# 123-code/Distributed-neural-networks

Measured on AMD Instinct MI355X. Metric: images/sec CIFAR-10 2-stage, higher is better.
Workload: dtype fp32 (bf16x3 split emulation, ~2^-16 per product); 1 GPU; model=cifar10-convnet (cifar_model_parts.py NeuralNetwork), global_batch=65536, parallelism=pp2-colocated, stages=2, microbatches=1, stage0_spare_cus=0, p2p=none, stage_cut=conv|fc (reference split, 16 KiB/img hop)

## Files before the change

csrc/bindings.cpp:

```cpp
#include <pybind11/pybind11.h>
#include <pybind11/stl.h>
#include <hip/hip_runtime.h>
#include <cstdint>

#include "kernels/api.h"
#include "comm/p2p.h"

#include <string>
#include <vector>

namespace py = pybind11;
#define P(x) reinterpret_cast<void*>(static_cast<uintptr_t>(x))
#define CP(x) reinterpret_cast<const void*>(static_cast<uintptr_t>(x))
#define FP(x) reinterpret_cast<float*>(static_cast<uintptr_t>(x))
#define CFP(x) reinterpret_cast<const float*>(static_cast<uintptr_t>(x))
#define IP(x) reinterpret_cast<int*>(static_cast<uintptr_t>(x))
#define CIP(x) reinterpret_cast<const int*>(static_cast<uintptr_t>(x))
#define ST(x) reinterpret_cast<hipStream_t>(static_cast<uintptr_t>(x))
typedef uint64_t u64;

PYBIND11_MODULE(_dnn_hip, m) {
  m.doc() = "distributed_neural_networks_amd HIP/CDNA4 kernels (gfx950)";
  m.attr("arch") = "gfx950";

// ... 62 lines not shown
                          int act, u64 qo, int ldq, u64 sxo, int kpo, u64 st) {
    return dnn_gemm_fp8_mx(CP(a), CP(sx), CP(w), CFP(sw), P(c), ldc, CFP(bias), CP(r), ldr, M, N, Kb, act, P(qo), ldq,
                           P(sxo), kpo, ST(st));
  });
  m.def("gemm_fp8_qkv_scatter_mx", [](u64 a, u64 sx, u64 w, u64 sw, u64 bias, u64 q, u64 kc, u64 vc, u64 pos, int B,
                                      int T, int H, int Hkv, int hd, int S, int Kb, u64 st) {
    return dnn_gemm_fp8_qkv_scatter_mx(CP(a), CP(sx), CP(w), CFP(sw), CFP(bias), P(q), P(kc), P(vc),
                                       reinterpret_cast<const int*>(static_cast<uintptr_t>(pos)), B, T, H, Hkv, hd, S,
                                       Kb, ST(st));
  });
  m.def("argmax_final", [](u64 part, int S, int M, u64 out, u64 out2, u64 pos_inc, u64 st, u64 hist, int hist_ld) {
    return dnn_argmax_final(CP(part), S, M, IP(out), IP(out2), IP(pos_inc), ST(st), IP(hist), hist_ld);
  });
  m.def("gemm_oneshot_sweep", [](u64 A, int lda, u64 Wsh, u64 sw, u64 C, int ldc, int M, int N, int K, int mt, int ntw,
                                 int steps, int splitk, int w8, u64 ws, long long ws_bytes, u64 st) {
    return dnn_gemm_oneshot_sweep(CP(A), lda, CP(Wsh), CFP(sw), P(C), ldc, M, N, K, mt, ntw, steps, splitk, w8, P(ws),
                                  ws_bytes, ST(st));
  });
  m.def("gemm_skinny_sweep", [](u64 A, int lda, u64 W, int ldw, u64 sw, u64 C, int ldc, int M, int N, int K, int nt,
                                int u, int ks, int pipe, int w8, u64 st) {
    return dnn_gemm_skinny_sweep(CP(A), lda, CP(W), ldw, CFP(sw), P(C), ldc, M, N, K, nt, u, ks, pipe, w8, ST(st));
  });
  m.def("gemm_set_tile", [](int tile) { return dnn_gemm_set_tile(tile); });
  m.def("gemm_set_anatomy", [](int bits) { return dnn_gemm_set_anatomy(bits); });
  m.def("gemm_set_skinny_pin", [](int id, int ks, int n, int k) { return dnn_gemm_set_skinny_pin(id, ks, n, k); });
  m.def("gemm_set_half_cost", [](float c) { return dnn_gemm_set_half_cost(c); });
  m.def("gemm_bf16_qkv_scatter", [](u64 A, int lda, u64 W, int ldw, u64 bias, u64 rowstat, u64 colsum, u64 q, u64 kc,
                                    u64 vc, u64 pos, int B, int T, int H, int Hkv, int hd, int S, int K, u64 st) {
    return dnn_gemm_bf16_qkv_scatter(CP(A), lda, CP(W), ldw, CFP(bias), CFP(rowstat), CFP(colsum), P(q), P(kc), P(vc),
                                     CIP(pos), B, T, H, Hkv, hd, S, K, ST(st));
  });
  m.def("gemm_fp8_qkv_scatter", [](u64 A8, u64 sa, u64 W8, u64 sw, u64 bias, u64 q, u64 kc, u64 vc, u64 pos, int B,
                                   int T, int H, int Hkv, int hd, int S, int Kb, u64 st) {
    return dnn_gemm_fp8_qkv_scatter(CP(A8), CFP(sa), CP(W8), CFP(sw), CFP(bias), P(q), P(kc), P(vc), CIP(pos), B, T, H,
                                    Hkv, hd, S, Kb, ST(st));
  });
  m.def("gemm_set_res_prefetch", [](int on) { return dnn_gemm_set_res_prefetch(on); });
  m.def("gemm_set_skinny_max_m", [](int m) { return dnn_gemm_set_skinny_max_m(m); });
  m.def("gemm_fp8_set_tile", [](int tile) { return dnn_gemm_fp8_set_tile(tile); });
  m.def("silu_mul_packed", [](u64 gu, int ld_in, u64 out, int ld_out, int M, int F, u64 st) {
    return dnn_silu_mul_packed(CP(gu), ld_in, P(out), ld_out, M, F, ST(st));
  });
  m.def("cifar_stage0_v4", [](u64 x, u64 out, u64 w1p, u64 b1, u64 w2p, u64 b2, int B, int grid, u64 st) {
    return dnn_cifar_stage0_v4(CFP(x), P(out), CP(w1p), CFP(b1), CP(w2p), CFP(b2), B, grid, ST(st));
  });
  m.def("cifar_set_v4_pt", [](int pt) { return dnn_cifar_set_v4_pt(pt); });
  m.def("cifar_stage0_x3", [](u64 x, u64 out, u64 w1h, u64 w1l, u64 b1, u64 w2h, u64 w2l, u64 b2, int B, int grid,
                              u64 st, int split_out) {
    return dnn_cifar_stage0_x3(CFP(x), FP(out), CP(w1h), CP(w1l), CFP(b1), CP(w2h), CP(w2l), CFP(b2), B, grid,
                               ST(st), split_out);
  }, py::arg("x"), py::arg("out"), py::arg("w1h"), py::arg("w1l"), py::arg("b1"), py::arg("w2h"), py::arg("w2l"),
        py::arg("b2"), py::arg("B"), py::arg("grid"), py::arg("st"), py::arg("split_out") = 0);
  m.def("cifar_s0_set_wide_store", [](int on) { return dnn_cifar_s0_set_wide_store(on); });
  m.def("cifar_split3", [](u64 a, int lda, u64 o, int ldo, int M, int K, u64 st, int blocked) {
    return dnn_cifar_split3(CFP(a), lda, P(o), ldo, M, K, ST(st), blocked);
  }, py::arg("a"), py::arg("lda"), py::arg("o"), py::arg("ldo"), py::arg("M"), py::arg("K"), py::arg("st"),
        py::arg("blocked") = 0);
  m.def("cifar_fc1_x3", [](u64 a, int lda, u64 wh, u64 wl, int ldw, u64 bias, u64 c, int ldc, int M, int N, int K,
                           u64 st, int a_split) {
    return dnn_cifar_fc1_x3(CFP(a), lda, CP(wh), CP(wl), ldw, CFP(bias), FP(c), ldc, M, N, K, ST(st), a_split);
  }, py::arg("a"), py::arg("lda"), py::arg("wh"), py::arg("wl"), py::arg("ldw"), py::arg("bias"), py::arg("c"),
        py::arg("ldc"), py::arg("M"), py::arg("N"), py::arg("K"), py::arg("st"), py::arg("a_split") = 0);
  m.def("cifar_split_blocked", [](u64 a, u64 o, int M, int K, int dir, u64 st) {
    return dnn_cifar_split_blocked(CFP(a), FP(o), M, K, dir, ST(st));
  });
  m.def("cifar_head_tail_x3", [](u64 hid, u64 w2h, u64 w2l, u64 b2, u64 probs, u64 pred, int B, u64 st) {
    return dnn_cifar_head_tail_x3(CFP(hid), CP(w2h), CP(w2l), CFP(b2), FP(probs), IP(pred), B, ST(st));
  });
  m.def("cifar_head_tail", [](u64 hid, u64 w2p, u64 b2, u64 probs, u64 pred, int B, u64 st) {
    return dnn_cifar_head_tail(CP(hid), CP(w2p), CFP(b2), FP(probs), IP(pred), B, ST(st));
  });
#ifdef DNN_HAVE_TRANSFORMER
  m.def("row_stats", [](u64 x, int ldx, u64 stats, int M, int N, float eps, int rms, u64 st) {
    return dnn_row_stats(CP(x), ldx, FP(stats), M, N, eps, rms, ST(st));
  });
  m.def("layernorm", [](u64 x, int ldx, u64 w, u64 b, u64 y, int ldy, int M, int N, float eps, int rms, u64 st) {
    return dnn_layernorm(CP(x), ldx, CFP(w), CFP(b), P(y), ldy, M, N, eps, rms, ST(st));
  });
  m.def("layernorm_q8", [](u64 x, int ldx, u64 w, u64 b, u64 q, int ldq, u64 sq, int M, int N, int kpad, float eps,
                           int rms, u64 st, int split) {
    return dnn_layernorm_q8(CP(x), ldx, CFP(w), CFP(b), P(q), ldq, FP(sq), M, N, kpad, eps, rms, ST(st), split);
  }, py::arg("x"), py::arg("ldx"), py::arg("w"), py::arg("b"), py::arg("q"), py::arg("ldq"), py::arg("sq"), py::arg("M"),
     py::arg("N"), py::arg("kpad"), py::arg("eps"), py::arg("rms"), py::arg("st"), py::arg("split") = 0);
  m.def("embed_gpt2", [](u64 idx, u64 wte, u64 wpe, u64 out, int B, int T, int d, u64 pos, int V, int Pn, u64 st) {
    return dnn_embed_gpt2(CIP(idx), CP(wte), CP(wpe), P(out), B, T, d, CIP(pos), V, Pn, ST(st));
  });
  m.def("qkv_split", [](u64 qkv, u64 q, u64 kc, u64 vc, int B, int T, int H, int Hkv, int hd, int S, u64 pos,
                        u64 cos, u64 sin, int rope, u64 st, int kv8) {
    return dnn_qkv_split(CP(qkv), P(q), P(kc), P(vc), B, T, H, Hkv, hd, S, CIP(pos), CFP(cos), CFP(sin), rope,
                         ST(st), kv8);
  }, py::arg("qkv"), py::arg("q"), py::arg("kc"), py::arg("vc"), py::arg("B"), py::arg("T"), py::arg("H"),
     py::arg("Hkv"), py::arg("hd"), py::arg("S"), py::arg("pos"), py::arg("cos"), py::arg("sin"), py::arg("rope"),
     py::arg("st"), py::arg("kv8") = 0);
  m.def("flash_attn_qkv", [](u64 qkv, int ldqkv, u64 kc, u64 vc, u64 o, int B, int T, int H, int Hkv, int hd, int S,
                             u64 pos, float scale, u64 st, int kv8) {
    return dnn_flash_attn_qkv(CP(qkv), ldqkv, P(kc), P(vc), P(o), B, T, H, Hkv, hd, S, CIP(pos), scale, ST(st), kv8);
  }, py::arg("qkv"), py::arg("ldqkv"), py::arg("kc"), py::arg("vc"), py::arg("o"), py::arg("B"), py::arg("T"),
     py::arg("H"), py::arg("Hkv"), py::arg("hd"), py::arg("S"), py::arg("pos"), py::arg("scale"), py::arg("st"),
     py::arg("kv8") = 0);
  m.def("flash_attn", [](u64 q, u64 kc, u64 vc, u64 o, int B, int T, int H, int Hkv, int hd, int S, u64 pos,
                         float scale, u64 st, int kv8) {
    return dnn_flash_attn(CP(q), CP(kc), CP(vc), P(o), B, T, H, Hkv, hd, S, CIP(pos), scale, ST(st), kv8);
  }, py::arg("q"), py::arg("kc"), py::arg("vc"), py::arg("o"), py::arg("B"), py::arg("T"), py::arg("H"),
     py::arg("Hkv"), py::arg("hd"), py::arg("S"), py::arg("pos"), py::arg("scale"), py::arg("st"), py::arg("kv8") = 0);
  m.def("attn_decode", [](u64 q, u64 kc, u64 vc, u64 o, int B, int H, int Hkv, int hd, int S, u64 lens,
                          float scale, int splits, u64 ws, u64 st, int kv8) {
// ... 79 lines not shown
```

csrc/kernels/api.h:

```cpp
#pragma once
#include <hip/hip_runtime.h>

extern "C" {
int dnn_gemm_bf16(const void* A, int lda, const void* W, int ldw, void* C, int ldc, const float* bias, const void* R,
                  int ldr, int M, int N, int K, int act, int out_f32, hipStream_t st, const void* Wsh = nullptr,
                  const float* rowstat = nullptr, const float* colsum = nullptr, void* ws = nullptr,
                  long long ws_bytes = 0);
int dnn_row_stats(const void* x, int ldx, float* stats, int M, int N, float eps, int rms, hipStream_t st);
int dnn_gemm_set_tile(int tile);
int dnn_gemm_set_anatomy(int bits);
int dnn_gemm_set_skinny_pin(int id, int ks, int n, int k);
int dnn_gemm_bf16_qkv_scatter(const void* A, int lda, const void* W, int ldw, const float* bias, const float* rowstat,
                              const float* colsum, void* q, void* kc, void* vc, const int* pos, int B, int T, int H,
                              int Hkv, int hd, int S, int K, hipStream_t st);
int dnn_gemm_fp8_qkv_scatter(const void* A8, const float* sa, const void* W8, const float* sw, const float* bias,
                             void* q, void* kc, void* vc, const int* pos, int B, int T, int H, int Hkv, int hd, int S,
                             int Kb, hipStream_t st);
int dnn_gemm_set_res_prefetch(int on);
int dnn_gemm_set_half_cost(float c);
int dnn_gemm_set_skinny_max_m(int m);
int dnn_gemm_fp8_set_tile(int tile);
int dnn_gemm_fp8_256(const void* A, const float* sa, const void* W, const float* sw, void* C, int ldc, const float* bias,
                     const void* R, int ldr, int M, int N, int Kb, int act, hipStream_t st);
int dnn_gemm_skinny_sweep(const void* A, int lda, const void* W, int ldw, const float* sw, void* C, int ldc, int M,
                          int N, int K, int nt, int u, int ks, int pipe, int w8, hipStream_t st);
int dnn_gemm_skinny_norm(const void* A, int lda, const void* W, int ldw, void* C, int ldc, const float* bias,
                         const void* R, int ldr, int M, int N, int K, int act, int norm, const float* colsum, float eps,
                         hipStream_t st, const void* Wsh = nullptr, void* ws = nullptr, long long ws_bytes = 0);
int dnn_gemm_skinny_w8(const void* A, int lda, const void* W, int ldw, const float* sw, void* C, int ldc,
                       const float* bias, const void* R, int ldr, int M, int N, int K, int act, int norm,
                       const float* colsum, float eps, hipStream_t st, const void* Wsh = nullptr, void* ws = nullptr,
                       long long ws_bytes = 0);
int dnn_gemm_skinny(const void* A, int lda, const float* sa, const void* W, int ldw, const float* sw, void* C, int ldc,
                    const float* bias, const void* R, int ldr, int M, int N, int K, int act, int out_f32, int fp8,
                    hipStream_t st, const void* Wsh = nullptr, void* ws = nullptr, long long ws_bytes = 0);
int dnn_gemm_set_stream(int on, long long min_bytes, int fold = -1);
int dnn_gemm_set_oneshot(int on, int mt, int ntw, int steps, int splitk);
int dnn_gemm_set_oneshot_lds_floor(int bytes);
int dnn_gemm_set_oneshot_probe(void* rec, int abl);
int dnn_gemm_oneshot_sweep(const void* A, int lda, const void* Wsh, const float* sw, void* C, int ldc, int M, int N,
                           int K, int mt, int ntw, int steps, int splitk, int w8, void* ws, long long ws_bytes,
                           hipStream_t st);
int dnn_gemm_set_head(int on);
int dnn_gemm_head(const void* A, int lda, const void* Wsh, const float* sw, const float* colsum, const float* bias,
                  float eps, int norm, void* C, int ldc, int M, int N, int K, int w8, void* part, int part_cap,
                  hipStream_t st);
int dnn_argmax_final(const void* part, int S, int M, int* out, int* out2, int* pos_inc, hipStream_t st,
                     int* hist = nullptr, int hist_ld = 0);
int dnn_gemm_set_split_tail(int on);
int dnn_quant_fp8_mx(const void* x, int ldx, void* q, int ldq, void* sx, int M, int K, int kpad, hipStream_t st);
int dnn_layernorm_q8_mx(const void* x, int ldx, const float* w, const float* b, void* q, int ldq, void* sx, int M,
                        int N, int kpad, float eps, int rms, hipStream_t st);
int dnn_gemm_fp8_mx(const void* A8, const void* sx, const void* W8, const float* sw, void* C, int ldc,
                    const float* bias, const void* R, int ldr, int M, int N, int Kb, int act, void* qo, int ldq,
                    void* sxo, int kpo, hipStream_t st);
int dnn_gemm_fp8_qkv_scatter_mx(const void* A8, const void* sx, const void* W8, const float* sw, const float* bias,
                                void* q, void* kc, void* vc, const int* pos, int B, int T, int H, int Hkv, int hd,
                                int S, int Kb, hipStream_t st);
int dnn_gemm_rowstats(void* out, int out_ld, const void* in, int in_ld);
int dnn_gemm_rowstats_written();
int dnn_gemm_set_epi_prefetch(int on);
int dnn_gemm_oneshot_ablate(const void* A, int lda, const void* Wsh, const float* sw, void* C, int ldc, int M, int N,
                            int K, int cfg, int abl, hipStream_t st);
int dnn_silu_mul_packed(const void* gu, int ld_in, void* out, int ld_out, int M, int F, hipStream_t st);
int dnn_cifar_stage0_v4(const float* x, void* out, const void* w1p, const float* b1, const void* w2p, const float* b2,
                        int B, int grid, hipStream_t st);
int dnn_cifar_set_v4_pt(int pt);
int dnn_cifar_stage0_x3(const float* x, float* out, const void* w1h, const void* w1l, const float* b1, const void* w2h,
                        const void* w2l, const float* b2, int B, int grid, hipStream_t st, int split_out = 0);
int dnn_cifar_s0_set_wide_store(int on);
int dnn_cifar_split3(const float* a, int lda, void* o, int ldo, int M, int K, hipStream_t st, int blocked = 0);
int dnn_cifar_fc1_x3(const float* A, int lda, const void* Wh, const void* Wl, int ldw, const float* bias, float* C,
                     int ldc, int M, int N, int K, hipStream_t st, int a_split = 0);
int dnn_cifar_split_blocked(const float* a, float* o, int M, int K, int dir, hipStream_t st);
int dnn_cifar_head_tail_x3(const float* hid, const void* w2h, const void* w2l, const float* b2, float* probs, int* pred,
                           int B, hipStream_t st);
int dnn_cifar_head_tail(const void* hid, const void* w2p, const float* b2, float* probs, int* pred, int B,
                        hipStream_t st);
int dnn_layernorm_q8(const void* x, int ldx, const float* w, const float* b, void* q, int ldq, float* sq, int M, int N,
                     int kpad, float eps, int rms, hipStream_t st, int split = 0);
int dnn_layernorm(const void* x, int ldx, const float* w, const float* b, void* y, int ldy, int M, int N, float eps,
                  int rms, hipStream_t st);
int dnn_embed_gpt2(const int* idx, const void* wte, const void* wpe, void* out, int B, int T, int d, const int* pos,
                   int V, int P, hipStream_t st);
int dnn_qkv_split(const void* qkv, void* q, void* kc, void* vc, int B, int T, int H, int Hkv, int hd, int S,
                  const int* pos, const float* cos, const float* sin, int rope, hipStream_t st, int kv8 = 0);
int dnn_flash_attn_qkv(const void* qkv, int ldqkv, void* kc, void* vc, void* o, int B, int T, int H, int Hkv,
                       int hd, int S, const int* pos, float scale, hipStream_t st, int kv8 = 0);
int dnn_flash_attn(const void* q, const void* kc, const void* vc, void* o, int B, int T, int H, int Hkv, int hd, int S,
                   const int* pos, float scale, hipStream_t st, int kv8 = 0);
int dnn_attn_decode_qkv(const void* qkv, int ldqkv, void* kc, void* vc, void* o, int B, int H, int Hkv, int hd, int S,
                        const int* pos, const float* cosT, const float* sinT, float scale, int splits, float* ws,
                        hipStream_t st, int kv8 = 0);
int dnn_attn_decode(const void* q, const void* kc, const void* vc, void* o, int B, int H, int Hkv, int hd, int S,
                    const int* lens, float scale, int splits, float* ws, hipStream_t st, int kv8 = 0);
int dnn_sample_topk(const void* x, int ld, int M, int N, int* out, float temperature, int topk, unsigned seed,
                    const int* step, hipStream_t st);
int dnn_argmax_rows(const void* x, int ld, int M, int N, int* out, int f32in, hipStream_t st, int* out2 = nullptr,
                    int* pos_inc = nullptr, void* part = nullptr, int* hist = nullptr, int hist_ld = 0);
int dnn_quant_fp8_rows(const void* x, int ldx, void* q, float* scale, int M, int K, int kpad, hipStream_t st,
                       int split = 0);
int dnn_gemm_fp8(const void* A, const float* sa, const void* W, const float* sw, void* C, int ldc, const float* bias,
                 const void* R, int ldr, int M, int N, int K, int act, hipStream_t st);
}
```

csrc/kernels/cifar_x3.hip:

```cpp
#include <type_traits>

#include "gemm_epilogue.h"

namespace dnn {
namespace x3 {

__device__ __forceinline__ void split2(float a, float b, uint32_t& hi, uint32_t& lo) {
  hi = pack2bf(a, b);
  const float ah = __uint_as_float(hi << 16), bh = __uint_as_float(hi & 0xffff0000u);
  lo = pack2bf(a - ah, b - bh);
}

__device__ __forceinline__ int dpp_xor1(int v) { return __builtin_amdgcn_mov_dpp(v, 0xB1, 0xF, 0xF, false); }
__device__ __forceinline__ int dpp_xor2(int v) { return __builtin_amdgcn_mov_dpp(v, 0x4E, 0xF, 0xF, false); }

constexpr int XW = 40;
constexpr int XPL = 34 * XW * 8;
constexpr int A1PL = 18 * 18 * 64;
constexpr int A1_OFF = 4 * XPL;
constexpr int LDS_BYTES = A1_OFF + 4 * A1PL;

__device__ __forceinline__ int xin_off(int k, int lo) { return ((k & 1) * 2 + lo) * XPL; }
__device__ __forceinline__ int a1_off(int k, int lo) { return A1_OFF + ((k & 1) * 2 + lo) * A1PL; }

template <int S, int I, int LO>
__device__ __forceinline__ constexpr int c2_imm() {
  return (8 * I + (S >> 1) % 3) * 64 + LO * A1PL;
}

template <int S>
__device__ __forceinline__ void c2_issue(const uint32_t (&b)[3][2], bf16x8 (&a)[4]) {
  constexpr int ky = (S >> 1) / 3, par = S & 1;
  asm volatile("ds_read_b128 %0, %1 offset:%2" : "=v"(a[0]) : "v"(b[ky][par]), "i"(c2_imm<S, 0, 0>()));
  asm volatile("ds_read_b128 %0, %1 offset:%2" : "=v"(a[1]) : "v"(b[ky][par]), "i"(c2_imm<S, 1, 0>()));
  asm volatile("ds_read_b128 %0, %1 offset:%2" : "=v"(a[2]) : "v"(b[ky][par]), "i"(c2_imm<S, 0, 1>()));
  asm volatile("ds_read_b128 %0, %1 offset:%2" : "=v"(a[3]) : "v"(b[ky][par]), "i"(c2_imm<S, 1, 1>()));
}

template <int S>
__device__ __forceinline__ void c2_step(const uint32_t (&b)[3][2], const bf16x8 (&wh)[18], const bf16x8 (&wl)[18],
                                        f32x16 (&acc)[2], bf16x8 (&cur)[4], bf16x8 (&nxt)[4]) {
  if constexpr (S + 1 < 18) {
    c2_issue<S + 1>(b, nxt);
    asm volatile("s_waitcnt lgkmcnt(4)" ::: "memory");
  } else {
    asm volatile("s_waitcnt lgkmcnt(0)" ::: "memory");
  }
  __builtin_amdgcn_sched_barrier(0);
  acc[0] = __builtin_amdgcn_mfma_f32_32x32x16_bf16(cur[0], wh[S], acc[0], 0, 0, 0);
  acc[1] = __builtin_amdgcn_mfma_f32_32x32x16_bf16(cur[1], wh[S], acc[1], 0, 0, 0);
  acc[0] = __builtin_amdgcn_mfma_f32_32x32x16_bf16(cur[0], wl[S], acc[0], 0, 0, 0);
  acc[1] = __builtin_amdgcn_mfma_f32_32x32x16_bf16(cur[1], wl[S], acc[1], 0, 0, 0);
  acc[0] = __builtin_amdgcn_mfma_f32_32x32x16_bf16(cur[2], wh[S], acc[0], 0, 0, 0);
  acc[1] = __builtin_amdgcn_mfma_f32_32x32x16_bf16(cur[3], wh[S], acc[1], 0, 0, 0);
  __builtin_amdgcn_sched_barrier(0);
  if constexpr (S + 1 < 18) c2_step<S + 1>(b, wh, wl, acc, nxt, cur);
}

template <int N>
__device__ __forceinline__ void resident_fence(const bf16x8 (&w)[N]) {
#pragma unroll
  for (int i = 0; i < N; ++i) asm volatile("" ::"v"(w[i]));
}

}

using namespace x3;

template <bool WIDE, bool SPLIT_OUT>
__global__ __launch_bounds__(512, 1) void cifar_stage0_x3_kernel(
    const float* __restrict__ x, float* __restrict__ out, const bf16_t* __restrict__ w1h,
    const bf16_t* __restrict__ w1l, const float* __restrict__ b1, const bf16_t* __restrict__ w2h,
    const bf16_t* __restrict__ w2l, const float* __restrict__ b2, int B) {
  __shared__ __attribute__((aligned(16))) char smem[LDS_BYTES];
  const int tid = threadIdx.x, lane = tid & 63;
  const int wave = __builtin_amdgcn_readfirstlane(tid >> 6);
  const bool producer = wave < 4;
  const int rw = wave & 3;
  const int rt = tid & 255;
  const int h = lane >> 5, r32 = lane & 31;
  const int n = B > (int)blockIdx.x ? (B - 1 - (int)blockIdx.x) / (int)gridDim.x + 1 : 0;

  for (int i = tid; i < LDS_BYTES / 16; i += 512) reinterpret_cast<uint4*>(smem)[i] = make_uint4(0, 0, 0, 0);

  __syncthreads();

  if (producer) {
    bf16x8 w1hf[3], w1lf[3];
#pragma unroll
    for (int s = 0; s < 3; ++s) {
      w1hf[s] = *reinterpret_cast<const bf16x8*>(w1h + r32 * 48 + s * 16 + h * 8);
      w1lf[s] = *reinterpret_cast<const bf16x8*>(w1l + r32 * 48 + s * 16 + h * 8);
    }
    const float bias = b1[r32];
    resident_fence(w1hf);
    resident_fence(w1lf);
    asm volatile("" ::"v"(bias));

    float pf[4][3];
    auto load_img = [&](int k) {
      const float* xb = x + (size_t)(blockIdx.x + (size_t)k * gridDim.x) * 3072;
#pragma unroll
      for (int i = 0; i < 4; ++i)
#pragma unroll
        for (int c = 0; c < 3; ++c) pf[i][c] = xb[c * 1024 + rt + 256 * i];
    };
    auto stage_img = [&](int k) {
      char* xh = smem + xin_off(k, 0);
      char* xl = smem + xin_off(k, 1);
#pragma unroll
      for (int i = 0; i < 4; ++i) {
        const int p = rt + 256 * i, yy = p >> 5, xx = p & 31;
        uint2 vh, vl;
        split2(pf[i][0], pf[i][1], vh.x, vl.x);
        split2(pf[i][2], 0.f, vh.y, vl.y);
        const int o = ((yy + 1) * XW + xx + 1) * 8;
        *reinterpret_cast<uint2*>(xh + o) = vh;
        *reinterpret_cast<uint2*>(xl + o) = vl;
      }
    };
    const int c1_lane = ((r32 >> 3) * XW + (r32 & 7) + 2 * h) * 8;
    const int q = ((r32 & 1) ? 2 : 0) + ((r32 & 2) ? 1 : 0);
    const int cb = r32 & ~3;

    auto conv1_epi = [&](int t, const f32x16& acc, int k) {
      const int ty = t >> 2, tx = t & 3;
      float v[4];
#pragma unroll
      for (int qy = 0; qy < 2; ++qy)
#pragma unroll
        for (int qx = 0; qx < 2; ++qx) {
          const int g0 = (2 * qy) * 4 + 2 * qx;
          v[qy * 2 + qx] = fmaxf(fmax_nan(fmax_nan(acc[g0], acc[g0 + 1]), fmax_nan(acc[g0 + 4], acc[g0 + 5])) + bias, 0.f);
        }
      const bool odd = r32 & 1;
      const int s0 = __float_as_int(odd ? v[0] : v[2]), s1 = __float_as_int(odd ? v[1] : v[3]);
      const float r0 = __int_as_float(dpp_xor1(s0)), r1 = __int_as_float(dpp_xor1(s1));
      uint32_t u0h, u0l, u1h, u1l;
      if (!odd) {
        split2(v[0], r0, u0h, u0l);
        split2(v[1], r1, u1h, u1l);
      } else {
        split2(r0, v[2], u0h, u0l);
        split2(r1, v[3], u1h, u1l);
      }
      const bool hi2 = r32 & 2;
      const uint32_t rch = (uint32_t)dpp_xor2((int)(hi2 ? u0h : u1h));
      const uint32_t rcl = (uint32_t)dpp_xor2((int)(hi2 ? u0l : u1l));
      const uint32_t mh = hi2 ? u1h : u0h, ml = hi2 ? u1l : u0l;
      uint2 wh, wl;
      wh.x = hi2 ? rch : mh;
      wh.y = hi2 ? mh : rch;
      wl.x = hi2 ? rcl : ml;
      wl.y = hi2 ? ml : rcl;
      const int Y = 2 * ty + (q >> 1) + 1, X = 4 * tx + 2 * h + (q & 1) + 1;
      const int o = (Y * 18 + X) * 64 + ((((cb >> 3) ^ (Y & 3))) << 4) + (cb & 7) * 2;
      *reinterpret_cast<uint2*>(smem + a1_off(k, 0) + o) = wh;
      *reinterpret_cast<uint2*>(smem + a1_off(k, 1) + o) = wl;
    };
    auto frag = [&](const char* p) {
      const uint2 a = *reinterpret_cast<const uint2*>(p);
      const uint2 b = *reinterpret_cast<const uint2*>(p + 8);
      return __builtin_bit_cast(bf16x8, make_uint4(a.x, a.y, b.x, b.y));
    };
    auto conv1_pair = [&](int ta, int tb, int k) {
      const char* xh = smem + xin_off(k, 0);
      const int oa = c1_lane + ((4 * (ta >> 2)) * XW + 8 * (ta & 3)) * 8;
      const int ob = c1_lane + ((4 * (tb >> 2)) * XW + 8 * (tb & 3)) * 8;
      bf16x8 fah[3], fal[3], fbh[3], fbl[3];
#pragma unroll
      for (int s = 0; s < 3; ++s) {
        fah[s] = frag(xh + oa + s * XW * 8);
        fbh[s] = frag(xh + ob + s * XW * 8);
        fal[s] = frag(xh + XPL + oa + s * XW * 8);
        fbl[s] = frag(xh + XPL + ob + s * XW * 8);
      }
      f32x16 acca = {}, accb = {};
#pragma unroll
      for (int s = 0; s < 3; ++s) {
        acca = __builtin_amdgcn_mfma_f32_32x32x16_bf16(fah[s], w1hf[s], acca, 0, 0, 0);
        accb = __builtin_amdgcn_mfma_f32_32x32x16_bf16(fbh[s], w1hf[s], accb, 0, 0, 0);
        acca = __builtin_amdgcn_mfma_f32_32x32x16_bf16(fah[s], w1lf[s], acca, 0, 0, 0);
        accb = __builtin_amdgcn_mfma_f32_32x32x16_bf16(fbh[s], w1lf[s], accb, 0, 0, 0);
        acca = __builtin_amdgcn_mfma_f32_32x32x16_bf16(fal[s], w1hf[s], acca, 0, 0, 0);
        accb = __builtin_amdgcn_mfma_f32_32x32x16_bf16(fbl[s], w1hf[s], accb, 0, 0, 0);
      }
      conv1_epi(ta, acca, k);
      conv1_epi(tb, accb, k);
    };

    if (n > 0) {
      load_img(0);
      stage_img(0);
      if (n > 1) load_img(1);
    }
    __syncthreads();
    for (int it = 0; it <= n; ++it) {
      if (it < n) {
#pragma unroll 1
        for (int t = rw; t < 32; t += 8) conv1_pair(t, t + 4, it);
        if (it + 1 < n) {
          stage_img(it + 1);
          if (it + 2 < n) load_img(it + 2);
        }
      }
      __syncthreads();
    }
  } else {
    const int oc2 = (rw & 1) * 32 + r32;
    bf16x8 w2hf[18], w2lf[18];
#pragma unroll
    for (int s = 0; s < 18; ++s) {
      w2hf[s] = *reinterpret_cast<const bf16x8*>(w2h + oc2 * 288 + s * 16 + h * 8);
      w2lf[s] = *reinterpret_cast<const bf16x8*>(w2l + oc2 * 288 + s * 16 + h * 8);
    }
    const float bias = b2[oc2];
    resident_fence(w2hf);
    resident_fence(w2lf);
    asm volatile("" ::"v"(bias));
    uint32_t lb[3][2];
#pragma unroll
    for (int ky = 0; ky < 3; ++ky)
#pragma unroll
      for (int par = 0; par < 2; ++par) {
        const int yr = (r32 >> 3) + ky;
        lb[ky][par] = (uint32_t)((yr * 18 + (r32 & 7)) * 64 + (((2 * par + h) ^ (yr & 3)) << 4));
      }

    auto conv2_img = [&](int k) {
      float* ob = out + (size_t)(blockIdx.x + (size_t)k * gridDim.x) * 4096 + oc2 * 64;
      const uint32_t plane = (uint32_t)(uintptr_t)(smem + a1_off(k, 0));
#pragma unroll 1
      for (int p = 0; p < 2; ++p) {
        const int ty2 = (rw >> 1) * 2 + p;
        const uint32_t rb = plane + ty2 * 4 * 18 * 64;
        uint32_t b[3][2];
#pragma unroll
        for (int ky = 0; ky < 3; ++ky)
#pragma unroll
          for (int par = 0; par < 2; ++par) b[ky][par] = rb + lb[ky][par];
        f32x16 acc[2] = {f32x16{}, f32x16{}};
        bf16x8 a0[4], a1[4];
        c2_issue<0>(b, a0);
        c2_step<0>(b, w2hf, w2lf, acc, a0, a1);
        if constexpr (WIDE) {
#pragma unroll
          for (int qy = 0; qy < 2; ++qy) {
            const int g0 = (2 * qy) * 4;
            float v[2][2];
#pragma unroll
            for (int i = 0; i < 2; ++i) {
              v[i][0] = fmaxf(fmax_nan(fmax_nan(acc[i][g0], acc[i][g0 + 1]), fmax_nan(acc[i][g0 + 4], acc[i][g0 + 5])) + bias, 0.f);
              v[i][1] = fmaxf(fmax_nan(fmax_nan(acc[i][g0 + 2], acc[i][g0 + 3]), fmax_nan(acc[i][g0 + 6], acc[i][g0 + 7])) + bias,
                              0.f);
            }
            const auto sx = __builtin_amdgcn_permlane32_swap(__float_as_uint(v[0][0]), __float_as_uint(v[1][0]), false,
                                                             false);
            const auto sy = __builtin_amdgcn_permlane32_swap(__float_as_uint(v[0][1]), __float_as_uint(v[1][1]), false,
// ... 280 lines not shown
  bf16x8 wfh[16], wfl[16];
#pragma unroll
  for (int s = 0; s < 16; ++s) {
    wfh[s] = *reinterpret_cast<const bf16x8*>(w2h + col * 512 + s * 32 + kq);
    wfl[s] = *reinterpret_cast<const bf16x8*>(w2l + col * 512 + s * 32 + kq);
  }
  const float bias = col < 10 ? b2[col] : 0.f;
  for (int r0 = gw * 16; r0 < B; r0 += nw * 16) {
    const int row = r0 + (lane & 15);
    const int rc = row < B ? row : B - 1;
    const float* ap = hid + (size_t)rc * 512 + kq;
    f32x4 acc = {0.f, 0.f, 0.f, 0.f};
#pragma unroll
    for (int s = 0; s < 16; ++s) {
      const float4 u = *reinterpret_cast<const float4*>(ap + s * 32);
      const float4 v = *reinterpret_cast<const float4*>(ap + s * 32 + 4);
      uint4 hi, lo;
      split2(u.x, u.y, hi.x, lo.x);
      split2(u.z, u.w, hi.y, lo.y);
      split2(v.x, v.y, hi.z, lo.z);
      split2(v.z, v.w, hi.w, lo.w);
      const bf16x8 ah = __builtin_bit_cast(bf16x8, hi), al = __builtin_bit_cast(bf16x8, lo);
      acc = __builtin_amdgcn_mfma_f32_16x16x32_bf16(ah, wfh[s], acc, 0, 0, 0);
      acc = __builtin_amdgcn_mfma_f32_16x16x32_bf16(ah, wfl[s], acc, 0, 0, 0);
      acc = __builtin_amdgcn_mfma_f32_16x16x32_bf16(al, wfh[s], acc, 0, 0, 0);
    }
#pragma unroll
    for (int r = 0; r < 4; ++r) {
      const float z = col < 10 ? acc[r] + bias : -INFINITY;
      float mx = z;
#pragma unroll
      for (int o = 1; o < 16; o <<= 1) mx = fmaxf(mx, __shfl_xor(mx, o, 64));
      const float e = col < 10 ? expf(z - mx) : 0.f;
      float sum = e;
#pragma unroll
      for (int o = 1; o < 16; o <<= 1) sum += __shfl_xor(sum, o, 64);
      int cand = (z == mx) ? col : 16;
#pragma unroll
      for (int o = 1; o < 16; o <<= 1) cand = min(cand, __shfl_xor(cand, o, 64));
      const int m = r0 + (lane >> 4) * 4 + r;
      if (m < B) {
        if (col < 10) probs[(size_t)m * 10 + col] = e / sum;
        if (col == 0) pred[m] = cand;
      }
    }
  }
}

}

using namespace dnn;

static int g_s0_wide_store = 1;

extern "C" int dnn_cifar_s0_set_wide_store(int on) {
  g_s0_wide_store = on ? 1 : 0;
  return 0;
}

template <bool SPLIT_OUT>
static int launch_stage0_x3(const float* x, float* out, const void* w1h, const void* w1l, const float* b1,
                            const void* w2h, const void* w2l, const float* b2, int B, int grid, hipStream_t st) {
  if (g_s0_wide_store)
    hipLaunchKernelGGL((cifar_stage0_x3_kernel<true, SPLIT_OUT>), dim3(grid), dim3(512), 0, st, x, out,
                       (const bf16_t*)w1h, (const bf16_t*)w1l, b1, (const bf16_t*)w2h, (const bf16_t*)w2l, b2, B);
  else
    hipLaunchKernelGGL((cifar_stage0_x3_kernel<false, SPLIT_OUT>), dim3(grid), dim3(512), 0, st, x, out,
                       (const bf16_t*)w1h, (const bf16_t*)w1l, b1, (const bf16_t*)w2h, (const bf16_t*)w2l, b2, B);
  return (int)hipGetLastError();
}

extern "C" int dnn_cifar_stage0_x3(const float* x, float* out, const void* w1h, const void* w1l, const float* b1,
                                   const void* w2h, const void* w2l, const float* b2, int B, int grid,
                                   hipStream_t st, int split_out) {
  if (B <= 0) return 0;
  if (grid <= 0) grid = 256;
  if (grid > B) grid = B;
  return split_out ? launch_stage0_x3<true>(x, out, w1h, w1l, b1, w2h, w2l, b2, B, grid, st)
                   : launch_stage0_x3<false>(x, out, w1h, w1l, b1, w2h, w2l, b2, B, grid, st);
}

extern "C" int dnn_cifar_fc1_x3(const float* A, int lda, const void* Wh, const void* Wl, int ldw, const float* bias,
                                float* C, int ldc, int M, int N, int K, hipStream_t st, int a_split) {
  if (M <= 0) return 0;
  if (N % F1_T != 0 || K % F1_K != 0 || lda % 4 != 0 || ldw % 8 != 0 || ldc % 4 != 0) return -1;
  const int blocks = ((M + F1_T - 1) / F1_T) * (N / F1_T);
  if (a_split)
    hipLaunchKernelGGL(cifar_fc1_x3_kernel<true>, dim3(blocks), dim3(512), 0, st, A, lda, (const bf16_t*)Wh,
                       (const bf16_t*)Wl, ldw, bias, C, ldc, M, N, K);
  else
    hipLaunchKernelGGL(cifar_fc1_x3_kernel<false>, dim3(blocks), dim3(512), 0, st, A, lda, (const bf16_t*)Wh,
                       (const bf16_t*)Wl, ldw, bias, C, ldc, M, N, K);
  return (int)hipGetLastError();
}

extern "C" int dnn_cifar_split_blocked(const float* a, float* o, int M, int K, int dir, hipStream_t st) {
  if (M <= 0) return 0;
  if (K % 32 != 0 || a == o) return -1;
  const long total = (long)M * (K / 8);
  long blocks = (total + 255) / 256;
  if (blocks > 8192) blocks = 8192;
  hipLaunchKernelGGL(cifar_split_blocked_kernel, dim3((int)blocks), dim3(256), 0, st, a, o, M, K, dir);
  return (int)hipGetLastError();
}

extern "C" int dnn_cifar_split3(const float* a, int lda, void* o, int ldo, int M, int K, hipStream_t st, int blocked) {
  if (M <= 0) return 0;
  if (K % 8 != 0 || lda % 4 != 0 || ldo % 8 != 0 || ldo < 3 * K || (blocked && K % 32 != 0)) return -1;
  const long total = (long)M * (K / 8);
  long blocks = (total + 255) / 256;
  if (blocks > 8192) blocks = 8192;
  hipLaunchKernelGGL(cifar_split3_kernel, dim3((int)blocks), dim3(256), 0, st, a, lda, (bf16_t*)o, ldo, M, K, blocked);
  return (int)hipGetLastError();
}

extern "C" int dnn_cifar_head_tail_x3(const float* hid, const void* w2h, const void* w2l, const float* b2,
// ... 10 lines not shown
```

distributed_neural_networks_amd/ops/cifar.py:

```python
from __future__ import annotations

from dataclasses import dataclass
from typing import Dict, Optional, Tuple

import torch

from ._lib import check, lib, ptr, stream_ptr
from .gemm import ACT_RELU, linear

PRECISIONS = ("fp32", "bf16")


def split_bf16(w: torch.Tensor) -> Tuple[torch.Tensor, torch.Tensor]:
    w = w.float()
    hi = w.to(torch.bfloat16)
    lo = (w - hi.float()).to(torch.bfloat16)
    return hi, lo


def _conv1_k48(sd) -> torch.Tensor:
    w = torch.zeros(32, 3, 4, 4)
    w[:, :, :3, :3] = sd["conv1.weight"].float().permute(0, 2, 3, 1)
    return w.reshape(32, 48)

# ... 41 lines not shown


def pack_stage0(sd: Dict[str, torch.Tensor], device, precision: str = "fp32") -> CifarStage0Weights:
    _check_precision(precision)
    b1 = sd["conv1.bias"].float().to(device).contiguous()
    b2 = sd["conv2.bias"].float().to(device).contiguous()
    w1, w2 = _conv1_k48(sd), _conv2_k288(sd)
    if precision == "bf16":
        return CifarStage0Weights("bf16", b1, b2,
                                  w1=w1.to(device=device, dtype=torch.bfloat16).contiguous(),
                                  w2=w2.to(device=device, dtype=torch.bfloat16).contiguous())
    (w1h, w1l), (w2h, w2l) = split_bf16(w1), split_bf16(w2)
    dv = lambda t: t.to(device).contiguous()
    return CifarStage0Weights("fp32", b1, b2, w1h=dv(w1h), w1l=dv(w1l), w2h=dv(w2h), w2l=dv(w2l))


def pack_head(sd: Dict[str, torch.Tensor], device, fc1: bool = True, fc2: bool = True,
              precision: str = "fp32") -> CifarHeadWeights:
    _check_precision(precision)
    w = CifarHeadWeights(precision)
    if fc1:
        f = sd["fc1.weight"].float()
        if precision == "bf16":
            w.w_fc1 = f.to(device=device, dtype=torch.bfloat16).contiguous()
        else:
            hi, lo = split_bf16(f)
            w.w_fc1 = torch.cat([hi, lo, hi], dim=1).to(device).contiguous()
            w.w_fc1h, w.w_fc1l = hi.to(device).contiguous(), lo.to(device).contiguous()
        w.b_fc1 = sd["fc1.bias"].float().to(device).contiguous()
    if fc2:
        f2 = _fc2_pad(sd)
        if precision == "bf16":
            w.w_fc2 = f2.to(device=device, dtype=torch.bfloat16).contiguous()
        else:
            hi, lo = split_bf16(f2)
            w.w_fc2h, w.w_fc2l = hi.to(device).contiguous(), lo.to(device).contiguous()
        w.b_fc2 = sd["fc2.bias"].float().to(device).contiguous()
    return w


def act_dtype(precision: str) -> torch.dtype:
    return torch.float32 if _check_precision(precision) == "fp32" else torch.bfloat16


STAGE0_GRID = 0
FC1_X3_MIN_ROWS = 16384


def set_stage0_grid(grid: int = 0) -> None:
    global STAGE0_GRID
    STAGE0_GRID = int(grid)


def _check_act(t: torch.Tensor, shape, dtype, what: str) -> None:
    if t.dtype != dtype or tuple(t.shape[1:]) != tuple(shape) or not t.is_contiguous():
        raise ValueError(f"{what}: expected contiguous {dtype} (B,{','.join(map(str, shape))}), "
                         f"got {t.dtype} {tuple(t.shape)}")


BOUNDARIES = ("fp32", "split")


def _split_boundary(boundary: str, precision: str) -> int:
    if boundary not in BOUNDARIES:
        raise ValueError(f"boundary must be one of {BOUNDARIES}, got {boundary!r}")
    if boundary == "split" and precision != "fp32":
        raise ValueError("the split boundary encoding exists for the fp32 precision only")
    return int(boundary == "split")


def encode_boundary(h: torch.Tensor, out: Optional[torch.Tensor] = None) -> torch.Tensor:
    out = torch.empty_like(h) if out is None else out
    check(lib().cifar_split_blocked(ptr(h), ptr(out), h.shape[0], h.shape[1], 0, stream_ptr()), "encode_boundary")
    return out


def decode_boundary(h: torch.Tensor, out: Optional[torch.Tensor] = None) -> torch.Tensor:
    out = torch.empty_like(h) if out is None else out
    check(lib().cifar_split_blocked(ptr(h), ptr(out), h.shape[0], h.shape[1], 1, stream_ptr()), "decode_boundary")
    return out


def stage0_forward(x: torch.Tensor, w: CifarStage0Weights, out: Optional[torch.Tensor] = None,
                   grid: int = 0, boundary: str = "fp32") -> torch.Tensor:
    split = _split_boundary(boundary, w.precision)
    grid = grid or STAGE0_GRID
    _check_act(x, (3, 32, 32), torch.float32, "stage0 input")
    B = x.shape[0]
    dt = act_dtype(w.precision)
    if out is None:
        out = torch.empty((B, 4096), dtype=dt, device=x.device)
    if tuple(out.shape) != (B, 4096) or out.dtype != dt or not out.is_contiguous():
        raise ValueError("stage0: bad output buffer")
    if w.precision == "fp32":
        check(lib().cifar_stage0_x3(ptr(x), ptr(out), ptr(w.w1h), ptr(w.w1l), ptr(w.b1), ptr(w.w2h), ptr(w.w2l),
                                    ptr(w.b2), B, grid, stream_ptr(), split), "cifar_stage0_x3")
    else:
        check(lib().cifar_stage0_v4(ptr(x), ptr(out), ptr(w.w1), ptr(w.b1), ptr(w.w2), ptr(w.b2), B, grid,
                                    stream_ptr()), "cifar_stage0_v4")
    return out


def fc1_forward(h: torch.Tensor, w: CifarHeadWeights, out: Optional[torch.Tensor] = None,
                scratch: Optional[torch.Tensor] = None, boundary: str = "fp32") -> torch.Tensor:
    split = _split_boundary(boundary, w.precision)
    dt = act_dtype(w.precision)
# ... 40 lines not shown
```

Baseline: 26.95 million images/s.

## Add 16x16x32 MFMA conv2 path for fp32 stage0 with register-resident weights

Adds a new conv2 code path in the stage0 x3 kernel that uses 16x16x32 bf16 MFMAs instead of the previous 32x32x16 shape. It keeps the hi/lo split weights resident in registers, software-pipelines LDS reads one tap ahead with explicit waitcnt, and changes the LDS swizzle to match the new read pattern. The epilogue fuses 2x2 max-pool through permlane16 swaps. This path is the default, so it trades higher register pressure and a different LDS swizzle for fewer LDS bytes per MFMA and better overlap.

```diff
diff --git a/csrc/bindings.cpp b/csrc/bindings.cpp
--- a/csrc/bindings.cpp
+++ b/csrc/bindings.cpp
@@ -138,6 +138,8 @@
   }, py::arg("x"), py::arg("out"), py::arg("w1h"), py::arg("w1l"), py::arg("b1"), py::arg("w2h"), py::arg("w2l"),
         py::arg("b2"), py::arg("B"), py::arg("grid"), py::arg("st"), py::arg("split_out") = 0);
   m.def("cifar_s0_set_wide_store", [](int on) { return dnn_cifar_s0_set_wide_store(on); });
+  m.def("cifar_s0_set_mfma", [](int v) { return dnn_cifar_s0_set_mfma(v); });
+  m.def("cifar_s0_get_mfma", []() { return dnn_cifar_s0_get_mfma(); });
   m.def("cifar_split3", [](u64 a, int lda, u64 o, int ldo, int M, int K, u64 st, int blocked) {
     return dnn_cifar_split3(CFP(a), lda, P(o), ldo, M, K, ST(st), blocked);
   }, py::arg("a"), py::arg("lda"), py::arg("o"), py::arg("ldo"), py::arg("M"), py::arg("K"), py::arg("st"),
diff --git a/csrc/kernels/api.h b/csrc/kernels/api.h
--- a/csrc/kernels/api.h
+++ b/csrc/kernels/api.h
@@ -69,6 +69,8 @@
 int dnn_cifar_stage0_x3(const float* x, float* out, const void* w1h, const void* w1l, const float* b1, const void* w2h,
                         const void* w2l, const float* b2, int B, int grid, hipStream_t st, int split_out = 0);
 int dnn_cifar_s0_set_wide_store(int on);
+int dnn_cifar_s0_set_mfma(int v);
+int dnn_cifar_s0_get_mfma();
 int dnn_cifar_split3(const float* a, int lda, void* o, int ldo, int M, int K, hipStream_t st, int blocked = 0);
 int dnn_cifar_fc1_x3(const float* A, int lda, const void* Wh, const void* Wl, int ldw, const float* bias, float* C,
                      int ldc, int M, int N, int K, hipStream_t st, int a_split = 0);
diff --git a/csrc/kernels/cifar_x3.hip b/csrc/kernels/cifar_x3.hip
--- a/csrc/kernels/cifar_x3.hip
+++ b/csrc/kernels/cifar_x3.hip
@@ -63,11 +63,75 @@
   for (int i = 0; i < N; ++i) asm volatile("" ::"v"(w[i]));
 }
 
+template <int C2>
+__device__ __forceinline__ int a1_swz(int Y) {
+  return C2 ? (2 * Y) & 3 : Y & 3;
+}
+
+template <int T, int J, int LO>
+__device__ __forceinline__ constexpr int m16_imm() {
+  return (((T >> 1) / 3) * 18 + 4 * (2 * (T & 1) + J) + (T >> 1) % 3) * 64 + LO * A1PL;
+}
+
+template <int T>
+__device__ __forceinline__ void m16_issue(const uint32_t (&b)[2], bf16x8 (&a)[4]) {
+  constexpr int kyp = ((T >> 1) / 3) & 1;
+  asm volatile("ds_read_b128 %0, %1 offset:%2" : "=v"(a[0]) : "v"(b[kyp]), "i"(m16_imm<T, 0, 0>()));
+  asm volatile("ds_read_b128 %0, %1 offset:%2" : "=v"(a[1]) : "v"(b[kyp]), "i"(m16_imm<T, 1, 0>()));
+  asm volatile("ds_read_b128 %0, %1 offset:%2" : "=v"(a[2]) : "v"(b[kyp]), "i"(m16_imm<T, 0, 1>()));
+  asm volatile("ds_read_b128 %0, %1 offset:%2" : "=v"(a[3]) : "v"(b[kyp]), "i"(m16_imm<T, 1, 1>()));
+}
+
+template <int T>
+__device__ __forceinline__ void m16_step(const uint32_t (&b)[2], const bf16x8 (&wh)[2][9], const bf16x8 (&wl)[2][9],
+                                         f32x4 (&acc)[4][2], bf16x8 (&cur)[4], bf16x8 (&nxt)[4]) {
+  constexpr int tap = T >> 1, m0 = 2 * (T & 1);
+  if constexpr (T + 1 < 18) {
+    m16_issue<T + 1>(b, nxt);
+    asm volatile("s_waitcnt lgkmcnt(4)" ::: "memory");
+  } else {
+    asm volatile("s_waitcnt lgkmcnt(0)" ::: "memory");
+  }
+  __builtin_amdgcn_sched_barrier(0);
+#pragma unroll
+  for (int term = 0; term < 3; ++term)
+#pragma unroll
+    for (int nt = 0; nt < 2; ++nt)
+#pragma unroll
+      for (int j = 0; j < 2; ++j)
+        acc[m0 + j][nt] = __builtin_amdgcn_mfma_f32_16x16x32_bf16(cur[(term == 2 ? 2 : 0) + j],
+                                                                  term == 1 ? wl[nt][tap] : wh[nt][tap], acc[m0 + j][nt], 0, 0, 0);
+  __builtin_amdgcn_sched_barrier(0);
+  if constexpr (T + 1 < 18) m16_step<T + 1>(b, wh, wl, acc, nxt, cur);
+}
+
+template <bool SPLIT_OUT, int NT>
+__device__ __forceinline__ void m16_epilogue(const f32x4 (&acc)[4][2], float bias, float* img, int oc, int PY, int x1) {
+  float v[4];
+#pragma unroll
+  for (int mt = 0; mt < 4; ++mt) {
+    const f32x4& a = acc[mt][NT];
+    v[mt] = fmaxf(fmax_nan(fmax_nan(a[0], a[1]), fmax_nan(a[2], a[3])) + bias, 0.f);
+  }
+  const auto s0 = __builtin_amdgcn_permlane16_swap(__float_as_uint(v[0]), __float_as_uint(v[2]), false, false);
+  const auto s1 = __builtin_amdgcn_permlane16_swap(__float_as_uint(v[1]), __float_as_uint(v[3]), false, false);
+  if constexpr (SPLIT_OUT) {
+    uint2 hi, lo;
+    split2(__uint_as_float(s0[0]), __uint_as_float(s0[1]), hi.x, lo.x);
+    split2(__uint_as_float(s1[0]), __uint_as_float(s1[1]), hi.y, lo.y);
+    char* bp = reinterpret_cast<char*>(img) + (oc * 2 + (PY >> 2)) * 128 + ((PY & 3) * 8 + 4 * x1) * 2;
+    *reinterpret_cast<uint2*>(bp) = hi;
+    *reinterpret_cast<uint2*>(bp + 64) = lo;
+  } else {
+    *reinterpret_cast<uint4*>(img + oc * 64 + PY * 8 + 4 * x1) = make_uint4(s0[0], s0[1], s1[0], s1[1]);
+  }
+}
+
 }
 
 using namespace x3;
 
-template <bool WIDE, bool SPLIT_OUT>
+template <bool WIDE, bool SPLIT_OUT, int C2 = 0>
 __global__ __launch_bounds__(512, 1) void cifar_stage0_x3_kernel(
     const float* __restrict__ x, float* __restrict__ out, const bf16_t* __restrict__ w1h,
     const bf16_t* __restrict__ w1l, const float* __restrict__ b1, const bf16_t* __restrict__ w2h,
@@ -154,7 +218,7 @@
       wl.x = hi2 ? rcl : ml;
       wl.y = hi2 ? ml : rcl;
       const int Y = 2 * ty + (q >> 1) + 1, X = 4 * tx + 2 * h + (q & 1) + 1;
-      const int o = (Y * 18 + X) * 64 + ((((cb >> 3) ^ (Y & 3))) << 4) + (cb & 7) * 2;
+      const int o = (Y * 18 + X) * 64 + ((((cb >> 3) ^ a1_swz<C2>(Y))) << 4) + (cb & 7) * 2;
       *reinterpret_cast<uint2*>(smem + a1_off(k, 0) + o) = wh;
       *reinterpret_cast<uint2*>(smem + a1_off(k, 1) + o) = wl;
     };
@@ -204,6 +268,52 @@
           if (it + 2 < n) load_img(it + 2);
         }
       }
+      __syncthreads();
+    }
+  } else if constexpr (C2 != 0) {
+    const int m = lane & 15, q16 = lane >> 4, y1 = q16 >> 1, x1 = q16 & 1;
+    const int oc = (rw & 1) * 32 + m;
+    bf16x8 w2hf[2][9], w2lf[2][9];
+#pragma unroll
+    for (int nt = 0; nt < 2; ++nt)
+#pragma unroll
+      for (int tap = 0; tap < 9; ++tap) {
+        w2hf[nt][tap] = *reinterpret_cast<const bf16x8*>(w2h + (oc + 16 * nt) * 288 + tap * 32 + q16 * 8);
+        w2lf[nt][tap] = *reinterpret_cast<const bf16x8*>(w2l + (oc + 16 * nt) * 288 + tap * 32 + q16 * 8);
+      }
+    const float bias0 = b2[oc], bias1 = b2[oc + 16];
+    resident_fence(w2hf[0]);
+    resident_fence(w2hf[1]);
+    resident_fence(w2lf[0]);
+    resident_fence(w2lf[1]);
+    asm volatile("" ::"v"(bias0), "v"(bias1));
+    const int py = 2 * (m >> 3) + ((m >> 1) & 1), px = 2 * ((m >> 2) & 1) + (m & 1);
+    uint32_t lb[2];
+#pragma unroll
+    for (int kyp = 0; kyp < 2; ++kyp) lb[kyp] = (uint32_t)((py * 18 + px) * 64 + ((q16 ^ a1_swz<C2>(py + kyp)) << 4));
+
+    auto conv2_img = [&](int k) {
+      float* img = out + (size_t)(blockIdx.x + (size_t)k * gridDim.x) * 4096;
+      const uint32_t plane = (uint32_t)(uintptr_t)(smem + a1_off(k, 0));
+#pragma unroll 1
+      for (int p = 0; p < 2; ++p) {
+        const int ty2 = (rw >> 1) * 2 + p;
+        const uint32_t rb = plane + ty2 * 4 * 18 * 64;
+        const uint32_t b[2] = {rb + lb[0], rb + lb[1]};
+        f32x4 acc[4][2];
+#pragma unroll
+        for (int mt = 0; mt < 4; ++mt) acc[mt][0] = acc[mt][1] = f32x4{};
+        bf16x8 a0[4], a1[4];
+        m16_issue<0>(b, a0);
+        m16_step<0>(b, w2hf, w2lf, acc, a0, a1);
+        m16_epilogue<SPLIT_OUT, 0>(acc, bias0, img, oc, 2 * ty2 + y1, x1);
+        m16_epilogue<SPLIT_OUT, 1>(acc, bias1, img, oc + 16, 2 * ty2 + y1, x1);
+      }
+    };
+
+    __syncthreads();
+    for (int it = 0; it <= n; ++it) {
+      if (it >= 1) conv2_img(it - 1);
       __syncthreads();
     }
   } else {
@@ -590,6 +700,15 @@
 using namespace dnn;
 
 static int g_s0_wide_store = 1;
+static int g_s0_mfma = 1;
+
+extern "C" int dnn_cifar_s0_set_mfma(int v) {
+  if (v < 0 || v > 1) return 1;
+  g_s0_mfma = v;
+  return 0;
+}
+
+extern "C" int dnn_cifar_s0_get_mfma() { return g_s0_mfma; }
 
 extern "C" int dnn_cifar_s0_set_wide_store(int on) {
   g_s0_wide_store = on ? 1 : 0;
@@ -599,7 +718,10 @@
 template <bool SPLIT_OUT>
 static int launch_stage0_x3(const float* x, float* out, const void* w1h, const void* w1l, const float* b1,
                             const void* w2h, const void* w2l, const float* b2, int B, int grid, hipStream_t st) {
-  if (g_s0_wide_store)
+  if (g_s0_mfma == 1)
+    hipLaunchKernelGGL((cifar_stage0_x3_kernel<true, SPLIT_OUT, 1>), dim3(grid), dim3(512), 0, st, x, out,
+                       (const bf16_t*)w1h, (const bf16_t*)w1l, b1, (const bf16_t*)w2h, (const bf16_t*)w2l, b2, B);
+  else if (g_s0_wide_store)
     hipLaunchKernelGGL((cifar_stage0_x3_kernel<true, SPLIT_OUT>), dim3(grid), dim3(512), 0, st, x, out,
                        (const bf16_t*)w1h, (const bf16_t*)w1l, b1, (const bf16_t*)w2h, (const bf16_t*)w2l, b2, B);
   else
diff --git a/distributed_neural_networks_amd/ops/cifar.py b/distributed_neural_networks_amd/ops/cifar.py
--- a/distributed_neural_networks_amd/ops/cifar.py
+++ b/distributed_neural_networks_amd/ops/cifar.py
@@ -117,6 +117,16 @@
     STAGE0_GRID = int(grid)
 
 
+STAGE0_MFMA = {"32x32x16": 0, "16x16x32": 1}
+
+
+def set_stage0_mfma(shape) -> int:
+    v = STAGE0_MFMA[shape] if isinstance(shape, str) else int(shape)
+    prev = lib().cifar_s0_get_mfma()
+    check(lib().cifar_s0_set_mfma(v), "cifar_s0_set_mfma")
+    return prev
+
+
 def _check_act(t: torch.Tensor, shape, dtype, what: str) -> None:
     if t.dtype != dtype or tuple(t.shape[1:]) != tuple(shape) or not t.is_contiguous():
         raise ValueError(f"{what}: expected contiguous {dtype} (B,{','.join(map(str, shape))}), "
```

Result: faster. 27.99 million images/s, median of 6 (+3.9%).
